# trifectatechfoundation/zlib-rs

Hardware: NVIDIA H100
Metric: deflate_level6_raw_input_throughput_silesia_small_tar (higher is better)
Workload: dtype u8

## Files before the change

zlib_rs_b200/csrc/zb_engine.cu:

```cuda
#include <cuda_runtime.h>
#include <stdio.h>
#include <stdlib.h>
#include <string.h>
#include <new>
#include "../../include/zb_engine.h"
#include "zb_kernels.cuh"
#include "zb_engine_internal.h"

namespace zb {

constexpr uint32_t kSlowSub9 = 24576;
constexpr uint32_t kTailTiles = 2;
constexpr uint32_t kTailSub = 512;

thread_local char g_err[256] = "";

static void set_err(const char *what, cudaError_t e)
{
    snprintf(g_err, sizeof g_err, "%s: %s", what, cudaGetErrorString(e));
}

#define CK(call)                                                  \
    do {                                                          \
        cudaError_t e_ = (call);                                  \
        if (e_ != cudaSuccess) { set_err(#call, e_); return ZB_E_CUDA; } \
    } while (0)

__global__ void k_match(JobBufs);
__global__ void k_skip(JobBufs);
__global__ void k_nxt(JobBufs);
__global__ void k_path_tiles(JobBufs);
__global__ void k_path_chain(JobBufs, uint32_t, uint32_t);
__global__ void k_path_groups(JobBufs, uint32_t, uint32_t, uint4 *, uint32_t *);
__global__ void k_path_chain2(JobBufs, uint32_t, uint32_t, const uint4 *, uint32_t *, uint32_t *);
__global__ void k_path_mark(JobBufs, const uint32_t *, const uint32_t *);
__global__ void k_iter_lists(JobBufs, uint32_t *, uint32_t *, uint32_t);
__global__ void k_emit(JobBufs);
__global__ void k_holes(JobBufs, uint32_t);
__global__ void k_holes_cmp(JobBufs, uint32_t, uint32_t);
__global__ void k_tail(JobBufs);
__global__ void k_block_hist(JobBufs, uint32_t *);
__global__ void k_build_blocks(JobBufs, const uint32_t *);
__global__ void k_scan_blocks(JobBufs);
__global__ void k_encode(JobBufs);
__global__ void k_finish(JobBufs, const uint32_t *);
__global__ void k_literal_syms(JobBufs);
__global__ void k_stored(JobBufs);
__global__ void k_links2_std(JobBufs, uint32_t);
__global__ void k_links2_roll(JobBufs, uint32_t);
__global__ void k_links_fix_std(JobBufs);
__global__ void k_links_fix_roll(JobBufs);
// ... 6 lines not shown
__global__ void k_links_dict_ghost_apply(JobBufs, const uint32_t *);
__global__ void k_bgzf_setup(BgzfJob, uint64_t);
__global__ void k_serial_low_members(JobBufs, BgzfJob);
__global__ void k_bgzf_medium(JobBufs, BgzfJob);
__global__ void k_bgzf_slow_steps(JobBufs, BgzfJob);
__global__ void k_bgzf_slow_walk(JobBufs, BgzfJob);
__global__ void k_bgzf_hist(JobBufs, BgzfJob, uint32_t *);
__global__ void k_bgzf_build(JobBufs, BgzfJob, const uint32_t *);
__global__ void k_bgzf_size(JobBufs, BgzfJob);
__global__ void k_bgzf_scan(JobBufs, BgzfJob);
__global__ void k_bgzf_encode(JobBufs, BgzfJob);
__global__ void k_bgzf_frame(JobBufs, BgzfJob);
__global__ void k_batch_stage(const uint8_t *, const uint64_t *, const uint8_t *, BgzfJob, uint8_t *, uint64_t);
__global__ void k_batch_dict_ghost(JobBufs, BgzfJob);

constexpr uint32_t kMatchSmemBytes = (kWSize + kMatchSub + 512) + (kWSize + kMatchSub) * 2 + ((kWSize + kMatchSub) / 32 + 1) * 4 * 4 + 8192;
constexpr uint32_t kPathSmemBytes = kPathTile * 4 * 3;
constexpr uint32_t kLinks2SmemBytes = 65536 * 2 + kLinkTile * 2 + kLinkTile + 64 + 2048;
constexpr uint32_t kSkipSmemBytes = 2 * kWSize * 2 + 2 * (2 * kWSize / 32) * 4 + 8192 + 64;
constexpr uint32_t kSlowSubMax = 24576;
constexpr uint32_t kSlowSmemBytes = (kWSize + kSlowSubMax + kSlowAhead) * 3;
constexpr uint32_t kChainSmemBytes = kChainChunkTiles * kPathHead * 8;
constexpr uint32_t kChain2MaxSmem = 200 * 1024;
constexpr uint32_t kSerialSmemBytes = (65536 + kWSize) * 2 + 35824 + 16;
constexpr uint32_t kSerialSmemQuick = 65536 * 2 + 65536 + 16;

int Engine::init(int dev)
{
    int n = 0;
    cudaError_t e = cudaGetDeviceCount(&n);
    if (e != cudaSuccess || n == 0) {
// ... 34 lines not shown
Engine::~Engine()
{
    if (device < 0) return;
    cudaSetDevice(device);
    for (auto &b : bufs) if (b.p) cudaFree(b.p);
    if (h_stage) cudaFreeHost(h_stage);
    if (h_info) cudaFreeHost(h_info);
    if (d_info) cudaFree(d_info);
    if (d_check) cudaFree(d_check);
    if (ev0) cudaEventDestroy(ev0);
    if (ev1) cudaEventDestroy(ev1);
    if (evf) cudaEventDestroy(evf);
    if (evt) cudaEventDestroy(evt);
    for (int i = 0; i < kUpChunks; i++) if (evc[i]) cudaEventDestroy(evc[i]);
    if (evk) cudaEventDestroy(evk);
    if (st2) cudaStreamDestroy(st2);
    if (st) cudaStreamDestroy(st);
}

void Engine::pbegin()
{
    if (!profile) return;
    if (!pev0) { cudaEventCreate(&pev0); cudaEventCreate(&pev1); }
    cudaEventRecord(pev0, st);
}

void Engine::pend(int phase, uint32_t nlaunch)
{
    if (!profile) return;
    cudaEventRecord(pev1, st);
// ... 119 lines not shown
    RES(S_SYMB, 40000 * 4, sym_base, uint32_t *)
    RES(S_BMAP, (size_t)nmt * 8192, bucket_map, uint32_t *)
    RES(S_LR, npad * 2, Lr, uint16_t *)
    RES(S_KEYS, npad * 2, keys, uint16_t *)
    RES(S_LLAST, (size_t)nmt * 65536 * 2, link_last, uint16_t *)
    RES(S_CSTATE, (size_t)(npt + 1) * 16, chain_state, uint4 *)
    uint32_t chainG = 16;
    while ((uint64_t)chainG * chainG < npt) chainG += 8;
    const uint32_t chain_groups = (npt + chainG - 1) / chainG;
    const uint32_t chain2_smem = chainG * kPathHead * 8 + chain_groups * kPathHead * 16 + chainG * 8;
    const bool chain2 = chain2_smem <= kChain2MaxSmem;
    if ((rc = reserve(S_GFN, (size_t)chain_groups * kPathHead * 16 + ((size_t)npt + 4) * 4, &p)) != ZB_OK) return rc;
    uint4 *d_gfn = static_cast<uint4 *>(p);
    uint32_t *d_mark_cnt = reinterpret_cast<uint32_t *>(d_gfn + (size_t)chain_groups * kPathHead);
    uint32_t *d_mark_list = d_mark_cnt + 4;
    auto launch_chain = [&](uint32_t first_tile) {
        if (chain2) {
            k_path_groups<<<chain_groups, 1024, chainG * kPathHead * 8, st>>>(jb, npt, chainG, d_gfn, d_mark_cnt);
            k_path_chain2<<<chain_groups, 1024, chain2_smem, st>>>(jb, npt, chainG, d_gfn, d_mark_list, d_mark_cnt);
            launches++;
        } else k_path_chain<<<1, 1024, kChainSmemBytes, st>>>(jb, npt, first_tile);
    };
    auto launch_mark = [&](uint32_t grid) {
        if (chain2) k_path_mark<<<grid < npt ? grid : npt, 1024, kPathSmemBytes, st>>>(jb, d_mark_list, d_mark_cnt);
        else k_path_mark<<<npt, 1024, kPathSmemBytes, st>>>(jb, nullptr, nullptr);
    };
    uint32_t *d_lists;
    const uint32_t max_list = N / 512 + 2;
    if ((rc = reserve(S_LISTS, ((size_t)max_list + npt + nmt + 8) * 4, &p)) != ZB_OK) return rc;
    d_lists = static_cast<uint32_t *>(p);
    RES(S_HDIFF, (size_t)nwords * 8, hdiff, uint32_t *)
    jb.hdiff_words = nwords;
    RES(S_HCOARSE, (size_t)(N >> 10) + 16, hcoarse, uint8_t *)
    RES(S_MCHG, (((size_t)N >> 8) + 16) * 4 + 64, mchg, uint8_t *)
    RES(S_BLOCKS, (size_t)max_blocks * sizeof(BlockDesc), blocks, BlockDesc *)
    RES(S_BBASE, (size_t)max_blocks * 4, block_base, uint32_t *)
    uint32_t *d_freq;
    if ((rc = reserve(S_FREQ, (size_t)max_blocks * 320 * 4, &p)) != ZB_OK) return rc;
    d_freq = static_cast<uint32_t *>(p);
    uint8_t *d_out;
    if (dst_dev && dst_cap >= out_cap) d_out = static_cast<uint8_t *>(dst);
    else { if ((rc = reserve(S_OUT, out_cap + 16, &p)) != ZB_OK) return rc; d_out = static_cast<uint8_t *>(p); }
    jb.out = d_out;
    jb.out_cap = out_cap;
    void *d_ck;
// ... 152 lines not shown
            if (!jb.slow_mode) CK(cudaMemcpyAsync(jb.Lr, jb.L, npad * 2, cudaMemcpyDeviceToDevice, st));
            pend(0, 1);
            if (jb.slow_mode) {
                if (n_in > 0) {
                    iters = 1;
                    pbegin();
                    if (jb.slow_mode == 2) k_rle<<<(N + 255) / 256, 256, 0, st>>>(jb);
                    else {
                        jb.match_sub = level >= 9 ? kSlowSub9 : level == 8 ? 4096u : 8192u;
                        k_slow<<<(N + jb.match_sub - 1) / jb.match_sub, 1024, (kWSize + jb.match_sub + kSlowAhead) * 3, st>>>(jb);
                    }
                    pend(1, 1);
                    if (profile) phase_ms[11] = phase_ms[1];
                    pbegin();
                    k_path_tiles<<<npt, 1024, kPathSmemBytes, st>>>(jb);
                    launch_chain(0);
                    launch_mark(npt);
                    pend(3, 3);
                    pbegin();
                    k_emit_slow<<<(N + 255) / 256, 256, 0, st>>>(jb);
                    pend(4, 1);
                    launches += 5;
                }
                pbegin();
                k_tail_slow<<<1, 32, 0, st>>>(jb);
                launches++;
                pend(5, 1);
            } else {
            if (jb.tail_start > 0) {
                uint32_t n_dirty = nmt;
                for (;;) {
                    iters++;
                    uint32_t mthreads = 1024;
                    if (iters == 1) jb.match_sub = 4096;
                    else if (n_dirty <= kTailTiles) { jb.match_sub = kTailSub; mthreads = 256; }
                    else {
                        const uint64_t per_cta = (uint64_t)n_dirty * kMatchTile / (4 * (uint64_t)device_sm_count());
                        jb.match_sub = per_cta >= 8192 ? 8192 : per_cta >= 4096 ? 4096 : per_cta >= 2048 ? 2048 : 1024;
                    }
                    uint32_t nsub = (N + jb.match_sub - 1) / jb.match_sub;
                    uint32_t n_ptiles = npt, first_ptile = 0;
                    jb.skip_list = nullptr;
                    jb.nxt_list = nullptr;
                    if (iters > 1) {
                        jb.skip_list = d_lists;
                        jb.nxt_list = d_lists + nmt + 8;
                        n_ptiles = h_info->n_ptiles ? h_info->n_ptiles : 1;
                        first_ptile = h_info->first_ptile;
                        nsub = (n_dirty ? n_dirty : 1) * (kMatchTile / jb.match_sub);
                        if (n_dirty) {
                            pbegin();
                            k_skip<<<n_dirty, 1024, kSkipSmemBytes, st>>>(jb);
                            pend(1, 1);
                            launches++;
                        }
                    }
                    const uint32_t msmem = (kWSize + jb.match_sub + 512) + (kWSize + jb.match_sub) * 2 +
                                           (iters > 1 ? ((kWSize + jb.match_sub) / 32 + 1) * 4 * 4 + 8192 : 64);
                    jb.use_bucket_map = iters > 1;
                    pbegin();
                    k_match<<<nsub, mthreads, msmem, st>>>(jb);
                    pend(1, 1);
                    if (profile && iters == 1) phase_ms[11] = phase_ms[1];
                    pbegin();
                    k_nxt<<<n_ptiles * (kPathTile / 1024), 1024, 0, st>>>(jb);
                    pend(2, 1);
                    pbegin();
                    k_path_tiles<<<n_ptiles, 1024, kPathSmemBytes, st>>>(jb);
                    launch_chain(first_ptile);
                    launch_mark(iters == 1 ? npt : 2 * n_ptiles + 16);
                    pend(3, 3);
                    pbegin();
                    k_holes<<<(nlists * kLongPerSub + 255) / 256, 256, 0, st>>>(jb, nlists);
                    k_holes_cmp<<<(nwords + 255) / 256, 256, 0, st>>>(jb, nwords, nmt);
                    pend(4, 2);
                    launches += 7;
                    k_iter_lists<<<1, 1024, 0, st>>>(jb, d_lists, d_lists + nmt + 8, npt);
                    launches++;
                    CK(cudaMemcpyAsync(h_info, d_info, sizeof(JobInfo), cudaMemcpyDeviceToHost, st));
                    CK(cudaStreamSynchronize(st));
                    if (h_info->error) { snprintf(g_err, sizeof g_err, "engine error flags 0x%x (parse)", h_info->error); return ZB_E_INTERNAL; }
                    if (getenv("ZB_DEBUG")) {
                        static unsigned long long last[3];
                        if (iters == 1) memset(last, 0, sizeof last);
                        const double ctas = (double)(h_info->dbg[0] - last[0]) + 1e-9;
                        fprintf(stderr, "iter %u dirty %u: ctas %llu stage %.1f walk %.1f kcyc/cta, holes_changed %u, sub %u first_tile %u chain %u\n",
                                iters, n_dirty, h_info->dbg[0] - last[0], (h_info->dbg[1] - last[1]) / 1e3 / ctas,
                                (h_info->dbg[2] - last[2]) / 1e3 / ctas, h_info->holes_changed, jb.match_sub, first_ptile, chain2 ? 2u : 1u);
                        memcpy(last, h_info->dbg, sizeof last);
                    }
                    if (!h_info->holes_changed) break;
                    n_dirty = h_info->n_dirty;
                    if (iters > N / 257u + 4096u) { snprintf(g_err, sizeof g_err, "hole iteration did not converge"); return ZB_E_INTERNAL; }
                }
            }
            CK(cudaEventRecord(evf, st));
            CK(cudaStreamWaitEvent(st2, evf, 0));
            k_tail<<<1, 32, 0, st2>>>(jb);
            launches++;
            CK(cudaEventRecord(evt, st2));
            if (jb.tail_start > 0) {
                pbegin();
                k_emit<<<(jb.tail_start + 255) / 256, 256, 0, st>>>(jb);
                launches++;
                pend(4, 1);
            }
            pbegin();
            CK(cudaStreamWaitEvent(st, evt, 0));
            pend(5, 1);
            }
        }
        CK(cudaMemcpyAsync(h_info, d_info, sizeof(JobInfo), cudaMemcpyDeviceToHost, st));
        CK(cudaStreamSynchronize(st));
        if (h_info->error) { snprintf(g_err, sizeof g_err, "engine error flags 0x%x (tail)", h_info->error); return ZB_E_INTERNAL; }
        const uint32_t nblocks = h_info->n_blocks;
        if (nblocks == 0 || nblocks > max_blocks) { snprintf(g_err, sizeof g_err, "bad block count %u", nblocks); return ZB_E_INTERNAL; }
        pbegin();
        k_block_hist<<<nblocks, 256, 0, st>>>(jb, d_freq);
        k_build_blocks<<<nblocks, 32, 0, st>>>(jb, d_freq);
        k_scan_blocks<<<1, 256, 0, st>>>(jb);
        pend(6, 3);
        pbegin();
        k_encode<<<nblocks, 1024, 0, st>>>(jb);
        k_finish<<<1, 32, 0, st>>>(jb, d_check);
        pend(7, 2);
        launches += 5;
    }
    CK(cudaMemcpyAsync(h_info, d_info, sizeof(JobInfo), cudaMemcpyDeviceToHost, st));
    CK(cudaStreamSynchronize(st));
    CK(cudaGetLastError());
    if (h_info->error) {
        if (h_info->error & 8u) return ZB_E_BUF;
        snprintf(g_err, sizeof g_err, "engine error flags 0x%x (encode)", h_info->error);
        return ZB_E_INTERNAL;
    }
    const uint64_t out_bytes = h_info->out_bytes;
    if (out_bytes > dst_cap) {
        res->out_bytes = out_bytes;
        return ZB_E_BUF;
    }
    if (d_out != dst) {
        pbegin();
        CK(cudaMemcpyAsync(dst, d_out, out_bytes, dst_dev ? cudaMemcpyDeviceToDevice : cudaMemcpyDeviceToHost, st));
        pend(10, 0);
    }
    CK(cudaEventRecord(ev1, st));
    CK(cudaStreamSynchronize(st));
    float ms = 0;
// ... 655 lines not shown
```

zlib_rs_b200/csrc/zb_engine_internal.h:

```cpp
#pragma once
#include <cuda_runtime.h>
#include <stddef.h>
#include <stdint.h>
#include <vector>
#include "../../include/zb_engine.h"
#include "zb_index.h"
#include "zb_kernels.cuh"

namespace zb {

extern thread_local char g_err[256];
size_t deflate_bound(size_t n);

enum { S_IN, S_L, S_HOLES, S_HOLESN, S_M, S_NXT, S_PEXIT, S_PCNT, S_SYMIDX, S_TENTRY, S_TSYMB, S_TDIRTY, S_SYMS, S_SYMB,
       S_BLOCKS, S_SCRATCH, S_FREQ, S_OUT, S_CK, S_INF0, S_INF1, S_PHEAD, S_SK, S_MARKN, S_LLIST, S_LCNT, S_BMAP, S_HDIFF, S_HCOARSE, S_CSTATE, S_LISTS, S_LR, S_LLAST, S_BBASE, S_MCHG, S_GFN, S_KEYS, S_SHARD,
       S_MEMT, S_MEMC,
       S_BGZF,
       S_BATCH,
       S_INDEX,
       S_INDEXW,
       S_COUNT };

struct ShardState {
    int phase = 0;
// ... 39 lines not shown
    Buf bufs[kSlots];
    void *h_stage = nullptr;
    size_t h_stage_cap = 0;
    JobInfo *h_info = nullptr, *d_info = nullptr;
    uint32_t *d_check = nullptr;
    void *d_inf_state = nullptr, *h_inf_state = nullptr;
    uint32_t launches = 0;
    uint8_t h_prime = 0;
    static constexpr int kPhases = 12;
    bool profile = false;
    float phase_ms[kPhases] = {0};
    uint32_t phase_launches[kPhases] = {0};
    cudaEvent_t pev0 = nullptr, pev1 = nullptr;
    void pbegin();
    void pend(int phase, uint32_t nlaunch);

    int init(int dev);
    int inflate_init();
    ~Engine();
    int reserve(int slot, size_t bytes, void **out);
    int stage(size_t bytes);
    int deflate(const void *src, size_t n, bool src_dev, void *dst, size_t dst_cap, bool dst_dev, int level, int strategy,
                int window_bits, uint32_t flags, zb_deflate_result *res, const void *dict = nullptr, size_t dict_len = 0);
    int deflate_bgzf(const void *src, size_t n, bool src_dev, void *dst, size_t dst_cap, bool dst_dev, int level, zb_deflate_result *res);
    int deflate_batch(const void *dict, size_t dict_len, const void *src, const uint64_t *src_off, size_t n_items, bool src_dev, void *dst,
                      size_t dst_cap, bool dst_dev, int level, int strategy, int window_bits, uint32_t flags, uint64_t *dst_off,
                      uint32_t *checks, zb_deflate_result *res);
    int members_reserve(JobBufs &jb, BgzfJob &bj, uint32_t nm, uint32_t S, size_t span, int level, size_t out_cap, uint32_t wrap,
                        uint32_t **d_freq);
    int members_launch(JobBufs &jb, BgzfJob &bj, int level, uint32_t *d_freq);
// ... 34 lines not shown
```

zlib_rs_b200/csrc/zb_kernels.cu:

```cuda
#include "zb_kernels.cuh"

namespace zb {

__constant__ HuffTables c_tab;

cudaError_t upload_tables()
{
    HuffTables t;
    init_tables(t);
    return cudaMemcpyToSymbol(c_tab, &t, sizeof t);
}

struct GAcc {
    const uint8_t *data;
    uint32_t N;
    const uint16_t *L;
    const uint32_t *holes;
    const uint32_t *M;
    uint32_t w = kWSize;
    __device__ __forceinline__ uint32_t byte(uint32_t y) const
    {
        while (y >= N) {
            if (y < 2 * w) return 0;
            y -= w;
// ... 154 lines not shown
}

__global__ void __launch_bounds__(1024) k_links2_std(JobBufs jb, uint32_t tile0) { links2_body<false>(jb, tile0); }
__global__ void __launch_bounds__(1024) k_links2_roll(JobBufs jb, uint32_t tile0) { links2_body<true>(jb, tile0); }
__global__ void __launch_bounds__(256) k_links_fix_std(JobBufs jb) { links_fix_body<false>(jb); }
__global__ void __launch_bounds__(256) k_links_fix_roll(JobBufs jb) { links_fix_body<true>(jb); }

constexpr uint32_t kSkipSpan = 2 * kWSize;
__global__ void __launch_bounds__(1024) k_skip(JobBufs jb)
{
    extern __shared__ __align__(16) uint8_t smem[];
    uint16_t *sL = reinterpret_cast<uint16_t *>(smem);
    uint32_t *sh = reinterpret_cast<uint32_t *>(smem + kSkipSpan * 2);
    uint32_t *sf = sh + kSkipSpan / 32;
    uint32_t *sbm = sf + kSkipSpan / 32;
    const uint32_t tile = jb.skip_list ? jb.skip_list[blockIdx.x] : blockIdx.x;
    const uint32_t ts = tile * kMatchTile;
    if (ts >= jb.N) return;
    const uint32_t te = min(ts + kMatchTile, jb.N);
    const uint32_t ws = ts >= kWSize ? ts - kWSize : 0;
    const uint32_t span = te - ws, tid = threadIdx.x;
    const uint32_t md = jb.wsize - kMinLookahead;
    {
        const uint4 *ls = reinterpret_cast<const uint4 *>(jb.L + ws);
        uint4 *ld = reinterpret_cast<uint4 *>(sL);
        for (uint32_t i = tid; i < (span + 7) / 8; i += 1024) ld[i] = ls[i];
        for (uint32_t i = tid; i < (span + 31) / 32; i += 1024) sh[i] = jb.holes[(ws >> 5) + i];
        const uint32_t *bm1 = jb.bucket_map + (size_t)tile * 2048, *bm0 = tile ? bm1 - 2048 : bm1;
        for (uint32_t i = tid; i < 2048; i += 1024) sbm[i] = bm0[i] | bm1[i];
    }
// ... 280 lines not shown
                        }
                    }
                }
            }
        }
    }
}

__global__ void __launch_bounds__(1024, 2) k_match(JobBufs jb)
{
    extern __shared__ __align__(16) uint8_t smem[];
    __shared__ uint32_t s_next;
    __shared__ __align__(8) unsigned long long s_mbar;
    const uint32_t sub = jb.match_sub;
    const uint32_t per_tile = kMatchTile / sub;
    const uint32_t ts = (jb.skip_list ? jb.skip_list[blockIdx.x / per_tile] * per_tile + blockIdx.x % per_tile : blockIdx.x) * sub;
    if (ts >= jb.N) return;
    {
        const uint32_t t0 = ts / kMatchTile, t1 = (min(ts + sub, jb.N) - 1) / kMatchTile;
        if (!jb.tile_dirty[t0] && !jb.tile_dirty[t1]) return;
    }
    const uint32_t data_bytes = kWSize + sub + 512;
    uint8_t *sdata = smem;
    uint16_t *sL = reinterpret_cast<uint16_t *>(smem + data_bytes);
    uint32_t *sh = reinterpret_cast<uint32_t *>(smem + data_bytes + (kWSize + sub) * 2);
    uint32_t *sbm = sh;
    const uint32_t wmax = (kWSize + sub) / 32 + 1;
    uint32_t *sdel = sbm + 2048, *pdel = sdel + wmax, *sadd = pdel + wmax, *padd = sadd + wmax;
    __shared__ uint32_t s_wsum[32];
    const uint32_t N = jb.N;
// ... 116 lines not shown
    }
}

constexpr uint32_t kMacroReach = 22016;

__device__ __forceinline__ bool path_tile_dirty(const JobBufs &jb, uint32_t pt)
{
    const uint32_t m0 = (pt * kPathTile) / kMatchTile;
    uint32_t m1 = ((pt + 1) * kPathTile + kMacroReach - 1) / kMatchTile;
    if (m1 >= jb.nmt) m1 = jb.nmt - 1;
    bool d = false;
    for (uint32_t m = m0; m <= m1; m++) d = d || jb.tile_dirty[m];
    return d;
}

__global__ void __launch_bounds__(1024) k_nxt(JobBufs jb)
{
    constexpr uint32_t per = kPathTile / 1024;
    const uint32_t tile = jb.nxt_list ? jb.nxt_list[blockIdx.x / per] : blockIdx.x / per;
    if (!path_tile_dirty(jb, tile)) return;
    const uint32_t p = tile * kPathTile + (blockIdx.x % per) * 1024 + threadIdx.x;
    if (p >= jb.tail_start) return;
    if (jb.use_bucket_map) {
        const uint32_t old = jb.nxt[p];
        const uint32_t b0 = p >> 6, b1 = min(p + (old & 0xffffu), jb.N) >> 6;
        bool chg = false;
        for (uint32_t b = b0; b <= b1; b++) chg = chg || jb.mchg[b];
        if (!chg) return;
    }
    GAcc a{jb.in, jb.N, jb.L, jb.holes, jb.M, jb.wsize};
    const uint32_t long_len = 16 * jb.lp.lazy;
    uint32_t ns = 0, nlong = 0, lpos = 0, llen = 0;
    auto see = [&](const Sym &s) {
// ... 49 lines not shown
            v.x = p < jb.tail_start ? jb.nxt[p] : t;
            v.y = p + 1 < jb.tail_start ? jb.nxt[p + 1] : t;
            v.z = p + 2 < jb.tail_start ? jb.nxt[p + 2] : t;
            v.w = t;
        }
        dst[g] = v;
    }
}

__global__ void __launch_bounds__(1024) k_path_tiles(JobBufs jb)
{
    extern __shared__ __align__(16) uint8_t smem[];
    uint32_t *nx = reinterpret_cast<uint32_t *>(smem);
    uint32_t *ex = nx + kPathTile;
    uint32_t *cn = ex + kPathTile;
    const uint32_t tile = jb.nxt_list ? jb.nxt_list[blockIdx.x] : blockIdx.x;
    const uint32_t tbeg = tile * kPathTile;
    if (!path_tile_dirty(jb, tile)) return;
    path_load(jb, tbeg, nx);
    __syncthreads();
    const uint32_t warp = threadIdx.x >> 5, lane = threadIdx.x & 31;
    constexpr uint32_t kExitSub = 1024, nsub = kPathTile / kExitSub;
    for (uint32_t s = warp; s < nsub; s += blockDim.x / 32) path_subtile(nx, ex, cn, s * kExitSub, (s + 1) * kExitSub, lane);
    __syncthreads();
    for (int32_t j = (int32_t)nsub - 2; j >= 0; j--) {
        for (uint32_t i = threadIdx.x; i < kExitSub; i += blockDim.x) {
            const uint32_t p = (uint32_t)j * kExitSub + i;
            uint32_t t = ex[p];
            if (!(t & kStuck) && t < kPathTile) { cn[p] += cn[t]; ex[p] = ex[t]; }
        }
// ... 6 lines not shown
        if (p < jb.tail_start) {
            jb.pexit[p] = xa;
            jb.pcnt[p] = cn[i];
        }
        if (i < kPathHead) jb.phead[(size_t)tile * kPathHead + i] = make_uint2(xa, cn[i]);
    }
}

constexpr uint32_t kChainChunk = kChainChunkTiles;
__global__ void __launch_bounds__(1024) k_path_chain(JobBufs jb, uint32_t ntiles, uint32_t first_tile)
{
    extern __shared__ __align__(16) uint8_t smem[];
    uint2 *hd = reinterpret_cast<uint2 *>(smem);
    __shared__ uint32_t s_e, s_base, s_done, s_tail;
    __shared__ uint32_t c_entry[kChainChunk], c_base[kChainChunk];
    if (threadIdx.x == 0) {
        if (first_tile == 0) { s_e = jb.start; s_base = 0; s_done = jb.tail_start == 0; s_tail = jb.start; }
        else { const uint4 v = jb.chain_state[first_tile]; s_e = v.x; s_base = v.y; s_done = v.z; s_tail = v.w; }
    }
    for (uint32_t t = threadIdx.x; t < first_tile; t += blockDim.x) jb.mark_needed[t] = 0;
    __syncthreads();
    for (uint32_t c0 = first_tile; c0 < ntiles; c0 += kChainChunk) {
        const uint32_t nt = min(kChainChunk, ntiles - c0);
        for (uint32_t i = threadIdx.x; i < nt * kPathHead; i += blockDim.x) hd[i] = jb.phead[(size_t)c0 * kPathHead + i];
        __syncthreads();
        if (threadIdx.x == 0) {
            uint32_t e = s_e, base = s_base;
            bool done = s_done != 0;
            uint32_t tail_entry = s_tail;
            for (uint32_t k = 0; k < nt; k++) {
// ... 271 lines not shown
                diff &= diff - 1;
                if (y + 4 <= jb.N) {
                    const uint8_t *q = jb.in + y;
                    const uint32_t h = hash_u32((uint32_t)q[0] | ((uint32_t)q[1] << 8) | ((uint32_t)q[2] << 16) | ((uint32_t)q[3] << 24));
                    atomicOr(&sb[h >> 5], 1u << (h & 31));
                }
            }
        }
        jb.holes_new[w] = 0;
    }
    __syncthreads();
    uint32_t *bm = jb.bucket_map + (size_t)((blockIdx.x * blockDim.x * 32) / kMatchTile) * 2048;
    for (uint32_t i = threadIdx.x; i < 2048; i += blockDim.x) if (sb[i]) atomicOr(&bm[i], sb[i]);
}

__global__ void __launch_bounds__(1024) k_iter_lists(JobBufs jb, uint32_t *skip_list, uint32_t *path_list, uint32_t npt)
{
    __shared__ uint32_t s_wsum[32], s_total, s_first;
    const uint32_t tid = threadIdx.x, lane = tid & 31, warp = tid >> 5;
    if (tid == 0) s_first = 0xffffffffu;
    uint32_t base = 0;
    for (int which = 0; which < 2; which++) {
        const uint32_t n = which ? npt : jb.nmt;
        uint32_t *out = which ? path_list : skip_list;
        base = 0;
        for (uint32_t c0 = 0; c0 < n; c0 += 1024) {
            const uint32_t i = c0 + tid;
            const bool d = i < n && (which ? path_tile_dirty(jb, i) : jb.tile_dirty[i] != 0);
            const uint32_t m = __ballot_sync(0xffffffffu, d);
            __syncthreads();
            if (lane == 0) s_wsum[warp] = __popc(m);
// ... 8 lines not shown
            }
            __syncthreads();
            if (d) {
                out[base + s_wsum[warp] + __popc(m & ((1u << lane) - 1u))] = i;
                if (which) atomicMin(&s_first, i);
            }
            base += s_total;
        }
        __syncthreads();
        if (tid == 0) {
            if (which) { jb.info->n_ptiles = base; jb.info->first_ptile = s_first == 0xffffffffu ? 0u : s_first; }
            else jb.info->n_dirty = base;
        }
        if (tid == 0 && base == 0) out[0] = 0;
    }
}

struct GAccW {
    GAcc g;
    uint32_t w;
    __device__ __forceinline__ uint32_t byte(uint32_t y) const
    {
        while (y >= g.N) {
            if (y < 2 * w) return 0;
            y -= w;
        }
        return g.data[y];
    }
    __device__ __forceinline__ uint32_t link(uint32_t y) const { return g.link(y); }
    __device__ __forceinline__ bool inserted(uint32_t y) const { return g.inserted(y); }
// ... 36 lines not shown
        if (s.dist == 0) atomicAdd(&lf[s.lc], 1u);
        else {
            atomicAdd(&lf[257 + c_tab.length_code[s.lc]], 1u);
            atomicAdd(&df[d_code(c_tab, s.dist - 1u)], 1u);
        }
    }
    __syncthreads();
    for (uint32_t i = threadIdx.x; i < kLCodes; i += blockDim.x) fb[i] = lf[i];
    if (threadIdx.x < kDCodes) fb[kLCodes + threadIdx.x] = df[threadIdx.x];
}

__global__ void __launch_bounds__(256) k_block_hist(JobBufs jb, uint32_t *freq )
{
    const uint32_t b = blockIdx.x;
    const uint32_t nsyms = jb.info->n_syms, nblocks = jb.info->n_blocks;
    const uint32_t begin = b * jb.block_syms;
    const uint32_t count = (b + 1 < nblocks) ? jb.block_syms : nsyms - begin;
    block_hist_body(jb.syms, begin, count, freq + b * 320);
    if (threadIdx.x == 0) {
        BlockDesc &bd = jb.blocks[b];
        const bool last = b + 1 == nblocks;
        bd.sym_begin = begin;
        bd.sym_count = count;
        bd.last = last && !jb.not_last;
        const uint32_t start = begin == 0 ? jb.start : sym_end(jb.syms[begin - 1]);
        const uint32_t end = last ? jb.N : sym_end(jb.syms[begin + count - 1]);
        bd.in_start = start;
        bd.in_len = end - start;
        uint32_t Bf;
        if (last) Bf = jb.info->final_base;
// ... 306 lines not shown
    const uint64_t w = pos >> 5;
    const uint32_t sh = (uint32_t)(pos & 31);
    atomicOr(&out32[w], (uint32_t)(val << sh));
    if (sh + n > 32) {
        atomicOr(&out32[w + 1], (uint32_t)(val >> (32 - sh)));
        if (sh + n > 64) atomicOr(&out32[w + 2], (uint32_t)(val >> (64 - sh)));
    }
}

constexpr uint32_t kScanChunk = 1024;
__global__ void __launch_bounds__(256) k_scan_blocks(JobBufs jb)
{
    __shared__ uint64_t s_bits[kScanChunk];
    __shared__ uint64_t s_base[kScanChunk];
    __shared__ uint64_t s_bit;
    const uint32_t nb = jb.info->n_blocks;
    if (threadIdx.x == 0) s_bit = 8ull * jb.hdr_len + jb.prime_bits;
    for (uint32_t c0 = 0; c0 < nb; c0 += kScanChunk) {
        const uint32_t nc = min(kScanChunk, nb - c0);
        for (uint32_t i = threadIdx.x; i < nc; i += blockDim.x) {
            const BlockDesc &bd = jb.blocks[c0 + i];
            s_bits[i] = bd.type == 0 ? (1ull << 63) | (uint16_t)bd.in_len : (uint64_t)bd.hdr_bits + bd.body_bits;
        }
        __syncthreads();
        if (threadIdx.x == 0) {
            uint64_t bit = s_bit;
            for (uint32_t i = 0; i < nc; i++) {
                s_base[i] = bit;
                const uint64_t v = s_bits[i];
                bit = (v >> 63) ? ((bit + 3 + 7) & ~7ull) + 32 + 8ull * (v & 0xffffu) : bit + v;
// ... 110 lines not shown
        __syncthreads();
        uint64_t pos = bd.bit_base + bd.hdr_bits + round_bits + (incl - mybits) + (warp ? warp_sum[warp - 1] : 0);
#pragma unroll
        for (uint32_t j = 0; j < kSymsPerThread; j++) {
            or_bits(out32, pos, vals[j], lens[j]);
            pos += lens[j];
        }
        round_bits += warp_sum[31];
        __syncthreads();
    }
    if (tid == blockDim.x - 1 && round_bits != bd.body_bits) atomicOr(error, 16u);
}

__global__ void __launch_bounds__(1024) k_encode(JobBufs jb)
{
    if (jb.info->error) return;
    encode_body(jb.blocks[blockIdx.x], jb.syms, jb.in, jb.out, &jb.info->error);
}

__global__ void __launch_bounds__(256) k_bgzf_hist(JobBufs jb, BgzfJob bj, uint32_t *freq)
{
    const uint32_t b = blockIdx.x, m = b / kBgzfMaxBlocks, k = b % kBgzfMaxBlocks;
    const JobInfo &mi = bj.minfo[m];
    const uint32_t nsyms = mi.n_syms, nblocks = mi.n_blocks;
    if (k >= nblocks) return;
    const uint32_t base = (uint32_t)bj.moff[m], len = bj.pstart + bj.mlen[m];
    const Sym *syms = jb.syms + base;
    const uint32_t begin = k * jb.block_syms;
    const uint32_t count = k + 1 < nblocks ? jb.block_syms : nsyms - begin;
    block_hist_body(syms, begin, count, freq + (size_t)b * 320);
    if (threadIdx.x == 0) {
// ... 104 lines not shown
```

zlib_rs_b200/csrc/zb_kernels.cuh:

```cuda
#pragma once
#include <cuda_runtime.h>
#include "zb_core.h"
#include "zb_huff.h"
#include "zb_slow.h"
#include "zb_bgzf.h"

namespace zb {

constexpr uint32_t kLinkTile = 32768;
constexpr uint32_t kMatchTile = 32768;
constexpr uint32_t kMatchSub = 8192;
constexpr uint32_t kPathTile = 16384;
constexpr uint32_t kPathSub = 256;
constexpr uint32_t kLongPerSub = 4;
constexpr uint32_t kPathHead = 64;
constexpr uint32_t kChainChunkTiles = 320;
constexpr uint32_t kNxtTail = 0x80000000u;
constexpr uint32_t kNxtLong = 0x40000000u;
constexpr uint32_t kNxtLong258 = 0x20000000u;
constexpr uint32_t kSymsPerThread = 16;
constexpr uint32_t kSlowAhead = 1024;

__device__ __forceinline__ uint32_t sld_u8(uint32_t a) { uint32_t v; asm volatile("ld.shared.u8 %0, [%1];" : "=r"(v) : "r"(a)); return v; }
__device__ __forceinline__ uint32_t sld_u16(uint32_t a) { uint32_t v; asm volatile("ld.shared.u16 %0, [%1];" : "=r"(v) : "r"(a)); return v; }
// ... 7 lines not shown
struct JobInfo {
    uint32_t n_mid_syms;
    uint32_t tail_entry;
    uint32_t n_syms;
    uint32_t final_base;
    uint32_t holes_changed;
    uint32_t n_dirty, n_ptiles, first_ptile;
    uint32_t n_blocks;
    uint32_t data_type;
    uint32_t error;
    uint64_t total_bits;
    uint64_t out_bytes;
    uint32_t adler;
    uint64_t marker_byte;
    unsigned long long dbg[3];
};

struct JobBufs {
    const uint8_t *in;
    uint32_t N;
    uint32_t start;
    uint32_t tail_start;
    uint16_t *L;
    uint16_t *SK;
    uint32_t *hdiff;
    uint32_t hdiff_words;
    uint8_t *hcoarse;
    uint8_t *mchg;
    uint32_t *holes;
    uint32_t *holes_new;
    uint32_t *M;
// ... 59 lines not shown
    uint64_t *moff;
    uint32_t *mlen;
    uint32_t *mcheck;
    uint32_t *mbytes;
    uint64_t *mout;
    uint32_t *mstored;
    JobInfo *minfo;
    BgzfCtl *ctl;
    uint32_t pstart;
    uint32_t fdict;
    const uint32_t *dictid;
};

cudaError_t upload_tables();
int device_sm_count();
cudaError_t launch_adler32(const uint8_t *d_buf, uint64_t len, uint32_t start, void *d_scratch, size_t scratch_bytes, uint32_t *d_out,
                           cudaStream_t st);
cudaError_t launch_crc32(const uint8_t *d_buf, uint64_t len, uint32_t start, void *d_scratch, size_t scratch_bytes, uint32_t *d_out,
                         cudaStream_t st);
cudaError_t launch_crc32_segments(const uint8_t *d_buf, const uint64_t *d_off, const uint32_t *d_len, uint32_t nseg, uint32_t *d_crc,
                                  cudaStream_t st);
cudaError_t launch_crc32_join(const uint32_t *d_crc, const uint32_t *d_len, const uint32_t *d_count, uint32_t *d_out, cudaStream_t st);
cudaError_t launch_adler32_segments(const uint8_t *d_buf, const uint64_t *d_off, const uint32_t *d_len, uint32_t nseg, uint32_t *d_adler,
                                    cudaStream_t st);

}
```

Measured before the change: 1.598.

## Run hole iteration loop on device via CUDA graph conditional nodes

Replaces the host-driven hole-refinement loop, which synchronised and copied JobInfo back after every iteration, with a cached CUDA graph. The graph uses a while-conditional node and per-match-class if-branches, and k_iter_lists sets the conditions on the device. It also removes the host sync before block encoding by launching the encode kernels with max_blocks and letting them early-exit based on device-side n_blocks. The trade-off is over-provisioned grids, since kernels are launched with upper-bound sizes and exit early, plus graph build cost whenever the key changes.

```diff
diff --git a/zlib_rs_b200/csrc/zb_engine.cu b/zlib_rs_b200/csrc/zb_engine.cu
--- a/zlib_rs_b200/csrc/zb_engine.cu
+++ b/zlib_rs_b200/csrc/zb_engine.cu
@@ -10,8 +10,6 @@
 namespace zb {
 
 constexpr uint32_t kSlowSub9 = 24576;
-constexpr uint32_t kTailTiles = 2;
-constexpr uint32_t kTailSub = 512;
 
 thread_local char g_err[256] = "";
 
@@ -34,7 +32,7 @@
 __global__ void k_path_groups(JobBufs, uint32_t, uint32_t, uint4 *, uint32_t *);
 __global__ void k_path_chain2(JobBufs, uint32_t, uint32_t, const uint4 *, uint32_t *, uint32_t *);
 __global__ void k_path_mark(JobBufs, const uint32_t *, const uint32_t *);
-__global__ void k_iter_lists(JobBufs, uint32_t *, uint32_t *, uint32_t);
+__global__ void k_iter_lists(JobBufs, uint32_t *, uint32_t *, uint32_t, IterCtl);
 __global__ void k_emit(JobBufs);
 __global__ void k_holes(JobBufs, uint32_t);
 __global__ void k_holes_cmp(JobBufs, uint32_t, uint32_t);
@@ -71,7 +69,11 @@
 __global__ void k_batch_stage(const uint8_t *, const uint64_t *, const uint8_t *, BgzfJob, uint8_t *, uint64_t);
 __global__ void k_batch_dict_ghost(JobBufs, BgzfJob);
 
-constexpr uint32_t kMatchSmemBytes = (kWSize + kMatchSub + 512) + (kWSize + kMatchSub) * 2 + ((kWSize + kMatchSub) / 32 + 1) * 4 * 4 + 8192;
+constexpr uint32_t match_smem(uint32_t sub, bool later)
+{
+    return (kWSize + sub + 512) + (kWSize + sub) * 2 + (later ? ((kWSize + sub) / 32 + 1) * 4 * 4 + 8192 : 64);
+}
+constexpr uint32_t kMatchSmemBytes = match_smem(kMatchSub, true);
 constexpr uint32_t kPathSmemBytes = kPathTile * 4 * 3;
 constexpr uint32_t kLinks2SmemBytes = 65536 * 2 + kLinkTile * 2 + kLinkTile + 64 + 2048;
 constexpr uint32_t kSkipSmemBytes = 2 * kWSize * 2 + 2 * (2 * kWSize / 32) * 4 + 8192 + 64;
@@ -136,6 +138,9 @@
     if (evt) cudaEventDestroy(evt);
     for (int i = 0; i < kUpChunks; i++) if (evc[i]) cudaEventDestroy(evc[i]);
     if (evk) cudaEventDestroy(evk);
+    if (hg_exec) cudaGraphExecDestroy(hg_exec);
+    if (hg) cudaGraphDestroy(hg);
+    if (hg_st) cudaStreamDestroy(hg_st);
     if (st2) cudaStreamDestroy(st2);
     if (st) cudaStreamDestroy(st);
 }
@@ -285,21 +290,95 @@
     uint4 *d_gfn = static_cast<uint4 *>(p);
     uint32_t *d_mark_cnt = reinterpret_cast<uint32_t *>(d_gfn + (size_t)chain_groups * kPathHead);
     uint32_t *d_mark_list = d_mark_cnt + 4;
-    auto launch_chain = [&](uint32_t first_tile) {
+    auto launch_chain = [&](const JobBufs &j, cudaStream_t s, uint32_t first_tile) {
         if (chain2) {
-            k_path_groups<<<chain_groups, 1024, chainG * kPathHead * 8, st>>>(jb, npt, chainG, d_gfn, d_mark_cnt);
-            k_path_chain2<<<chain_groups, 1024, chain2_smem, st>>>(jb, npt, chainG, d_gfn, d_mark_list, d_mark_cnt);
-            launches++;
-        } else k_path_chain<<<1, 1024, kChainSmemBytes, st>>>(jb, npt, first_tile);
+            k_path_groups<<<chain_groups, 1024, chainG * kPathHead * 8, s>>>(j, npt, chainG, d_gfn, d_mark_cnt);
+            k_path_chain2<<<chain_groups, 1024, chain2_smem, s>>>(j, npt, chainG, d_gfn, d_mark_list, d_mark_cnt);
+        } else k_path_chain<<<1, 1024, kChainSmemBytes, s>>>(j, npt, first_tile);
     };
-    auto launch_mark = [&](uint32_t grid) {
-        if (chain2) k_path_mark<<<grid < npt ? grid : npt, 1024, kPathSmemBytes, st>>>(jb, d_mark_list, d_mark_cnt);
-        else k_path_mark<<<npt, 1024, kPathSmemBytes, st>>>(jb, nullptr, nullptr);
+    auto launch_mark = [&](const JobBufs &j, cudaStream_t s, uint32_t grid) {
+        if (chain2) k_path_mark<<<grid < npt ? grid : npt, 1024, kPathSmemBytes, s>>>(j, d_mark_list, d_mark_cnt);
+        else k_path_mark<<<npt, 1024, kPathSmemBytes, s>>>(j, nullptr, nullptr);
     };
     uint32_t *d_lists;
     const uint32_t max_list = N / 512 + 2;
     if ((rc = reserve(S_LISTS, ((size_t)max_list + npt + nmt + 8) * 4, &p)) != ZB_OK) return rc;
     d_lists = static_cast<uint32_t *>(p);
+    const uint32_t max_iters = N / 257u + 4096u;
+    bool graph_iters = false;
+    auto hole_graph = [&](uint32_t sms) -> int {
+        JobBufs jg = jb;
+        jg.out = nullptr;
+        jg.out_cap = 0;
+        jg.skip_list = d_lists;
+        jg.nxt_list = d_lists + nmt + 8;
+        jg.use_bucket_map = 1;
+        jg.match_sub = 0;
+        HoleGraphKey key;
+        memset(&key, 0, sizeof key);
+        key.jb = jg;
+        key.npt = npt; key.nlists = nlists; key.nwords = nwords; key.sms = sms; key.chain2 = chain2;
+        key.lists = d_lists; key.gfn = d_gfn;
+        if (hg_valid && memcmp(&key, &hg_key, sizeof key) == 0) return ZB_OK;
+        hg_valid = false;
+        if (hg_exec) { cudaGraphExecDestroy(hg_exec); hg_exec = nullptr; }
+        if (hg) { cudaGraphDestroy(hg); hg = nullptr; }
+        if (!hg_st) CK(cudaStreamCreateWithFlags(&hg_st, cudaStreamNonBlocking));
+        IterCtl ctl{};
+        ctl.graph = 1;
+        ctl.sms = sms;
+        ctl.max_iters = max_iters;
+        uint32_t dmax[kMatchClasses] = {1, 1, 1, 1, 1};
+        for (uint32_t d = 1; d <= nmt; d++) { const int c = match_class(d, sms); if (d > dmax[c]) dmax[c] = d; }
+        const uint32_t reach = path_tiles_per_match_tile(nmt, npt);
+        for (int c = 0; c < kMatchClasses; c++) ctl.ptile_bound[c] = (uint64_t)dmax[c] * reach < npt ? dmax[c] * reach : npt;
+        CK(cudaGraphCreate(&hg, 0));
+        cudaGraphConditionalHandle h;
+        CK(cudaGraphConditionalHandleCreate(&h, hg, 1, cudaGraphCondAssignDefault));
+        ctl.loop = h;
+        cudaGraphNodeParams wp = {cudaGraphNodeTypeConditional};
+        wp.conditional.handle = h;
+        wp.conditional.type = cudaGraphCondTypeWhile;
+        wp.conditional.size = 1;
+        cudaGraphNode_t node;
+        CK(cudaGraphAddNode(&node, hg, nullptr, 0, &wp));
+        cudaGraph_t body = wp.conditional.phGraph_out[0];
+        for (int c = 0; c < kMatchClasses; c++) {
+            CK(cudaGraphConditionalHandleCreate(&h, body, 0, cudaGraphCondAssignDefault));
+            ctl.cls[c] = h;
+        }
+        CK(cudaStreamBeginCaptureToGraph(hg_st, body, nullptr, nullptr, 0, cudaStreamCaptureModeThreadLocal));
+        k_iter_lists<<<1, 1024, 0, hg_st>>>(jg, d_lists, d_lists + nmt + 8, npt, ctl);
+        CK(cudaStreamEndCapture(hg_st, &body));
+        cudaGraphNode_t lists_node;
+        size_t nn = 1;
+        CK(cudaGraphGetNodes(body, &lists_node, &nn));
+        for (int c = 0; c < kMatchClasses; c++) {
+            cudaGraphNodeParams ip = {cudaGraphNodeTypeConditional};
+            ip.conditional.handle = ctl.cls[c];
+            ip.conditional.type = cudaGraphCondTypeIf;
+            ip.conditional.size = 1;
+            CK(cudaGraphAddNode(&node, body, &lists_node, 1, &ip));
+            cudaGraph_t br = ip.conditional.phGraph_out[0];
+            JobBufs jc = jg;
+            jc.match_sub = match_class_sub(c);
+            const uint32_t D = dmax[c], P = ctl.ptile_bound[c];
+            CK(cudaStreamBeginCaptureToGraph(hg_st, br, nullptr, nullptr, 0, cudaStreamCaptureModeThreadLocal));
+            k_skip<<<D, 1024, kSkipSmemBytes, hg_st>>>(jc);
+            k_match<<<D * (kMatchTile / jc.match_sub), c == 0 ? 256 : 1024, match_smem(jc.match_sub, true), hg_st>>>(jc);
+            k_nxt<<<P * (kPathTile / 1024), 1024, 0, hg_st>>>(jc);
+            k_path_tiles<<<P, 1024, kPathSmemBytes, hg_st>>>(jc);
+            launch_chain(jc, hg_st, kFirstFromInfo);
+            launch_mark(jc, hg_st, 2 * P + 16);
+            k_holes<<<(nlists * kLongPerSub + 255) / 256, 256, 0, hg_st>>>(jc, nlists);
+            k_holes_cmp<<<(nwords + 255) / 256, 256, 0, hg_st>>>(jc, nwords, nmt);
+            CK(cudaStreamEndCapture(hg_st, &br));
+        }
+        CK(cudaGraphInstantiate(&hg_exec, hg, 0));
+        hg_key = key;
+        hg_valid = true;
+        return ZB_OK;
+    };
     RES(S_HDIFF, (size_t)nwords * 8, hdiff, uint32_t *)
     jb.hdiff_words = nwords;
     RES(S_HCOARSE, (size_t)(N >> 10) + 16, hcoarse, uint8_t *)
@@ -482,8 +561,9 @@
                     if (profile) phase_ms[11] = phase_ms[1];
                     pbegin();
                     k_path_tiles<<<npt, 1024, kPathSmemBytes, st>>>(jb);
-                    launch_chain(0);
-                    launch_mark(npt);
+                    launch_chain(jb, st, 0);
+                    launch_mark(jb, st, npt);
+                    if (chain2) launches++;
                     pend(3, 3);
                     pbegin();
                     k_emit_slow<<<(N + 255) / 256, 256, 0, st>>>(jb);
@@ -496,15 +576,17 @@
                 pend(5, 1);
             } else {
             if (jb.tail_start > 0) {
+                const bool host_loop = profile || getenv("ZB_DEBUG") != nullptr;
+                const uint32_t sms = (uint32_t)device_sm_count();
                 uint32_t n_dirty = nmt;
                 for (;;) {
                     iters++;
                     uint32_t mthreads = 1024;
                     if (iters == 1) jb.match_sub = 4096;
-                    else if (n_dirty <= kTailTiles) { jb.match_sub = kTailSub; mthreads = 256; }
                     else {
-                        const uint64_t per_cta = (uint64_t)n_dirty * kMatchTile / (4 * (uint64_t)device_sm_count());
-                        jb.match_sub = per_cta >= 8192 ? 8192 : per_cta >= 4096 ? 4096 : per_cta >= 2048 ? 2048 : 1024;
+                        const int c = match_class(n_dirty, sms);
+                        jb.match_sub = match_class_sub(c);
+                        if (c == 0) mthreads = 256;
                     }
                     uint32_t nsub = (N + jb.match_sub - 1) / jb.match_sub;
                     uint32_t n_ptiles = npt, first_ptile = 0;
@@ -523,11 +605,9 @@
                             launches++;
                         }
                     }
-                    const uint32_t msmem = (kWSize + jb.match_sub + 512) + (kWSize + jb.match_sub) * 2 +
-                                           (iters > 1 ? ((kWSize + jb.match_sub) / 32 + 1) * 4 * 4 + 8192 : 64);
                     jb.use_bucket_map = iters > 1;
                     pbegin();
-                    k_match<<<nsub, mthreads, msmem, st>>>(jb);
+                    k_match<<<nsub, mthreads, match_smem(jb.match_sub, iters > 1), st>>>(jb);
                     pend(1, 1);
                     if (profile && iters == 1) phase_ms[11] = phase_ms[1];
                     pbegin();
@@ -535,15 +615,16 @@
                     pend(2, 1);
                     pbegin();
                     k_path_tiles<<<n_ptiles, 1024, kPathSmemBytes, st>>>(jb);
-                    launch_chain(first_ptile);
-                    launch_mark(iters == 1 ? npt : 2 * n_ptiles + 16);
+                    launch_chain(jb, st, first_ptile);
+                    launch_mark(jb, st, iters == 1 ? npt : 2 * n_ptiles + 16);
                     pend(3, 3);
                     pbegin();
                     k_holes<<<(nlists * kLongPerSub + 255) / 256, 256, 0, st>>>(jb, nlists);
                     k_holes_cmp<<<(nwords + 255) / 256, 256, 0, st>>>(jb, nwords, nmt);
                     pend(4, 2);
-                    launches += 7;
-                    k_iter_lists<<<1, 1024, 0, st>>>(jb, d_lists, d_lists + nmt + 8, npt);
+                    launches += chain2 ? 8 : 7;
+                    if (!host_loop) break;
+                    k_iter_lists<<<1, 1024, 0, st>>>(jb, d_lists, d_lists + nmt + 8, npt, IterCtl{});
                     launches++;
                     CK(cudaMemcpyAsync(h_info, d_info, sizeof(JobInfo), cudaMemcpyDeviceToHost, st));
                     CK(cudaStreamSynchronize(st));
@@ -559,7 +640,12 @@
                     }
                     if (!h_info->holes_changed) break;
                     n_dirty = h_info->n_dirty;
-                    if (iters > N / 257u + 4096u) { snprintf(g_err, sizeof g_err, "hole iteration did not converge"); return ZB_E_INTERNAL; }
+                    if (iters > max_iters) { snprintf(g_err, sizeof g_err, "hole iteration did not converge"); return ZB_E_INTERNAL; }
+                }
+                if (!host_loop) {
+                    if ((rc = hole_graph(sms)) != ZB_OK) return rc;
+                    CK(cudaGraphLaunch(hg_exec, st));
+                    graph_iters = true;
                 }
             }
             CK(cudaEventRecord(evf, st));
@@ -578,18 +664,13 @@
             pend(5, 1);
             }
         }
-        CK(cudaMemcpyAsync(h_info, d_info, sizeof(JobInfo), cudaMemcpyDeviceToHost, st));
-        CK(cudaStreamSynchronize(st));
-        if (h_info->error) { snprintf(g_err, sizeof g_err, "engine error flags 0x%x (tail)", h_info->error); return ZB_E_INTERNAL; }
-        const uint32_t nblocks = h_info->n_blocks;
-        if (nblocks == 0 || nblocks > max_blocks) { snprintf(g_err, sizeof g_err, "bad block count %u", nblocks); return ZB_E_INTERNAL; }
         pbegin();
-        k_block_hist<<<nblocks, 256, 0, st>>>(jb, d_freq);
-        k_build_blocks<<<nblocks, 32, 0, st>>>(jb, d_freq);
+        k_block_hist<<<max_blocks, 256, 0, st>>>(jb, d_freq);
+        k_build_blocks<<<max_blocks, 32, 0, st>>>(jb, d_freq);
         k_scan_blocks<<<1, 256, 0, st>>>(jb);
         pend(6, 3);
         pbegin();
-        k_encode<<<nblocks, 1024, 0, st>>>(jb);
+        k_encode<<<max_blocks, 1024, 0, st>>>(jb);
         k_finish<<<1, 32, 0, st>>>(jb, d_check);
         pend(7, 2);
         launches += 5;
@@ -597,9 +678,15 @@
     CK(cudaMemcpyAsync(h_info, d_info, sizeof(JobInfo), cudaMemcpyDeviceToHost, st));
     CK(cudaStreamSynchronize(st));
     CK(cudaGetLastError());
+    if (graph_iters) {
+        iters = h_info->iters;
+        launches += 1 + (iters - 1) * (chain2 ? 10u : 9u);
+    }
     if (h_info->error) {
         if (h_info->error & 8u) return ZB_E_BUF;
-        snprintf(g_err, sizeof g_err, "engine error flags 0x%x (encode)", h_info->error);
+        if (h_info->error & kErrNoConverge) snprintf(g_err, sizeof g_err, "hole iteration did not converge");
+        else if (h_info->error & kErrBlockCount) snprintf(g_err, sizeof g_err, "bad block count %u", h_info->n_blocks);
+        else snprintf(g_err, sizeof g_err, "engine error flags 0x%x", h_info->error);
         return ZB_E_INTERNAL;
     }
     const uint64_t out_bytes = h_info->out_bytes;
diff --git a/zlib_rs_b200/csrc/zb_engine_internal.h b/zlib_rs_b200/csrc/zb_engine_internal.h
--- a/zlib_rs_b200/csrc/zb_engine_internal.h
+++ b/zlib_rs_b200/csrc/zb_engine_internal.h
@@ -77,6 +77,16 @@
     cudaEvent_t pev0 = nullptr, pev1 = nullptr;
     void pbegin();
     void pend(int phase, uint32_t nlaunch);
+    struct HoleGraphKey {
+        JobBufs jb;
+        uint32_t npt, nlists, nwords, sms, chain2;
+        const void *lists, *gfn;
+    };
+    HoleGraphKey hg_key;
+    bool hg_valid = false;
+    cudaGraph_t hg = nullptr;
+    cudaGraphExec_t hg_exec = nullptr;
+    cudaStream_t hg_st = nullptr;
 
     int init(int dev);
     int inflate_init();
diff --git a/zlib_rs_b200/csrc/zb_kernels.cu b/zlib_rs_b200/csrc/zb_kernels.cu
--- a/zlib_rs_b200/csrc/zb_kernels.cu
+++ b/zlib_rs_b200/csrc/zb_kernels.cu
@@ -1,3 +1,4 @@
+#include <vector>
 #include "zb_kernels.cuh"
 
 namespace zb {
@@ -192,6 +193,7 @@
     uint32_t *sh = reinterpret_cast<uint32_t *>(smem + kSkipSpan * 2);
     uint32_t *sf = sh + kSkipSpan / 32;
     uint32_t *sbm = sf + kSkipSpan / 32;
+    if (jb.skip_list && blockIdx.x >= jb.info->n_dirty) return;
     const uint32_t tile = jb.skip_list ? jb.skip_list[blockIdx.x] : blockIdx.x;
     const uint32_t ts = tile * kMatchTile;
     if (ts >= jb.N) return;
@@ -502,6 +504,7 @@
     __shared__ __align__(8) unsigned long long s_mbar;
     const uint32_t sub = jb.match_sub;
     const uint32_t per_tile = kMatchTile / sub;
+    if (jb.skip_list && blockIdx.x / per_tile >= max(jb.info->n_dirty, 1u)) return;
     const uint32_t ts = (jb.skip_list ? jb.skip_list[blockIdx.x / per_tile] * per_tile + blockIdx.x % per_tile : blockIdx.x) * sub;
     if (ts >= jb.N) return;
     {
@@ -648,9 +651,23 @@
     return d;
 }
 
+uint32_t path_tiles_per_match_tile(uint32_t nmt, uint32_t npt)
+{
+    std::vector<uint32_t> cover(nmt, 0);
+    for (uint32_t pt = 0; pt < npt; pt++) {
+        const uint32_t m0 = (uint32_t)((uint64_t)pt * kPathTile / kMatchTile);
+        const uint32_t m1 = (uint32_t)(((uint64_t)(pt + 1) * kPathTile + kMacroReach - 1) / kMatchTile);
+        for (uint32_t m = m0; m <= m1 && m < nmt; m++) cover[m]++;
+    }
+    uint32_t most = 1;
+    for (uint32_t v : cover) most = v > most ? v : most;
+    return most;
+}
+
 __global__ void __launch_bounds__(1024) k_nxt(JobBufs jb)
 {
     constexpr uint32_t per = kPathTile / 1024;
+    if (jb.nxt_list && blockIdx.x / per >= max(jb.info->n_ptiles, 1u)) return;
     const uint32_t tile = jb.nxt_list ? jb.nxt_list[blockIdx.x / per] : blockIdx.x / per;
     if (!path_tile_dirty(jb, tile)) return;
     const uint32_t p = tile * kPathTile + (blockIdx.x % per) * 1024 + threadIdx.x;
@@ -730,6 +747,7 @@
     uint32_t *nx = reinterpret_cast<uint32_t *>(smem);
     uint32_t *ex = nx + kPathTile;
     uint32_t *cn = ex + kPathTile;
+    if (jb.nxt_list && blockIdx.x >= max(jb.info->n_ptiles, 1u)) return;
     const uint32_t tile = jb.nxt_list ? jb.nxt_list[blockIdx.x] : blockIdx.x;
     const uint32_t tbeg = tile * kPathTile;
     if (!path_tile_dirty(jb, tile)) return;
@@ -766,6 +784,7 @@
     uint2 *hd = reinterpret_cast<uint2 *>(smem);
     __shared__ uint32_t s_e, s_base, s_done, s_tail;
     __shared__ uint32_t c_entry[kChainChunk], c_base[kChainChunk];
+    if (first_tile == kFirstFromInfo) first_tile = jb.info->first_ptile;
     if (threadIdx.x == 0) {
         if (first_tile == 0) { s_e = jb.start; s_base = 0; s_done = jb.tail_start == 0; s_tail = jb.start; }
         else { const uint4 v = jb.chain_state[first_tile]; s_e = v.x; s_base = v.y; s_done = v.z; s_tail = v.w; }
@@ -1067,7 +1086,7 @@
     for (uint32_t i = threadIdx.x; i < 2048; i += blockDim.x) if (sb[i]) atomicOr(&bm[i], sb[i]);
 }
 
-__global__ void __launch_bounds__(1024) k_iter_lists(JobBufs jb, uint32_t *skip_list, uint32_t *path_list, uint32_t npt)
+__global__ void __launch_bounds__(1024) k_iter_lists(JobBufs jb, uint32_t *skip_list, uint32_t *path_list, uint32_t npt, IterCtl ctl)
 {
     __shared__ uint32_t s_wsum[32], s_total, s_first;
     const uint32_t tid = threadIdx.x, lane = tid & 31, warp = tid >> 5;
@@ -1106,6 +1125,15 @@
         }
         if (tid == 0 && base == 0) out[0] = 0;
     }
+    if (tid != 0) return;
+    const uint32_t iters = ++jb.info->iters;
+    if (!ctl.graph) return;
+    bool go = jb.info->holes_changed != 0;
+    if (go && iters > ctl.max_iters) { atomicOr(&jb.info->error, kErrNoConverge); go = false; }
+    const int c = match_class(jb.info->n_dirty, ctl.sms);
+    if (go && max(jb.info->n_ptiles, 1u) > ctl.ptile_bound[c]) { atomicOr(&jb.info->error, kErrListBound); go = false; }
+    cudaGraphSetConditional(ctl.loop, go ? 1u : 0u);
+    for (int k = 0; k < kMatchClasses; k++) cudaGraphSetConditional(ctl.cls[k], go && k == c ? 1u : 0u);
 }
 
 struct GAccW {
@@ -1172,6 +1200,9 @@
 {
     const uint32_t b = blockIdx.x;
     const uint32_t nsyms = jb.info->n_syms, nblocks = jb.info->n_blocks;
+    const bool bad = nblocks == 0 || nblocks > gridDim.x;
+    if (bad && b == 0 && threadIdx.x == 0) atomicOr(&jb.info->error, kErrBlockCount);
+    if (bad || b >= nblocks || jb.info->error) return;
     const uint32_t begin = b * jb.block_syms;
     const uint32_t count = (b + 1 < nblocks) ? jb.block_syms : nsyms - begin;
     block_hist_body(jb.syms, begin, count, freq + b * 320);
@@ -1508,6 +1539,7 @@
     __shared__ uint64_t s_bits[kScanChunk];
     __shared__ uint64_t s_base[kScanChunk];
     __shared__ uint64_t s_bit;
+    if (jb.info->error) return;
     const uint32_t nb = jb.info->n_blocks;
     if (threadIdx.x == 0) s_bit = 8ull * jb.hdr_len + jb.prime_bits;
     for (uint32_t c0 = 0; c0 < nb; c0 += kScanChunk) {
@@ -1648,7 +1680,7 @@
 
 __global__ void __launch_bounds__(1024) k_encode(JobBufs jb)
 {
-    if (jb.info->error) return;
+    if (jb.info->error || blockIdx.x >= jb.info->n_blocks) return;
     encode_body(jb.blocks[blockIdx.x], jb.syms, jb.in, jb.out, &jb.info->error);
 }
 
diff --git a/zlib_rs_b200/csrc/zb_kernels.cuh b/zlib_rs_b200/csrc/zb_kernels.cuh
--- a/zlib_rs_b200/csrc/zb_kernels.cuh
+++ b/zlib_rs_b200/csrc/zb_kernels.cuh
@@ -45,7 +45,32 @@
     uint32_t adler;
     uint64_t marker_byte;
     unsigned long long dbg[3];
+    uint32_t iters;
 };
+constexpr uint32_t kErrBlockCount = 64u;
+constexpr uint32_t kErrNoConverge = 256u;
+constexpr uint32_t kErrListBound = 512u;
+
+constexpr uint32_t kTailTiles = 2;
+constexpr uint32_t kTailSub = 512;
+constexpr int kMatchClasses = 5;
+__host__ __device__ inline int match_class(uint32_t n_dirty, uint32_t sms)
+{
+    if (n_dirty <= kTailTiles) return 0;
+    const uint64_t per_cta = (uint64_t)n_dirty * kMatchTile / (4 * (uint64_t)sms);
+    return per_cta >= 8192 ? 4 : per_cta >= 4096 ? 3 : per_cta >= 2048 ? 2 : 1;
+}
+__host__ __device__ inline uint32_t match_class_sub(int c) { return 512u << c; }
+
+struct IterCtl {
+    uint32_t graph;
+    uint32_t sms;
+    uint32_t max_iters;
+    uint32_t ptile_bound[kMatchClasses];
+    unsigned long long loop;
+    unsigned long long cls[kMatchClasses];
+};
+constexpr uint32_t kFirstFromInfo = 0xffffffffu;
 
 struct JobBufs {
     const uint8_t *in;
@@ -135,6 +160,7 @@
 
 cudaError_t upload_tables();
 int device_sm_count();
+uint32_t path_tiles_per_match_tile(uint32_t nmt, uint32_t npt);
 cudaError_t launch_adler32(const uint8_t *d_buf, uint64_t len, uint32_t start, void *d_scratch, size_t scratch_bytes, uint32_t *d_out,
                            cudaStream_t st);
 cudaError_t launch_crc32(const uint8_t *d_buf, uint64_t len, uint32_t start, void *d_scratch, size_t scratch_bytes, uint32_t *d_out,
```

New measurement: 1.601 (median of 6 runs). No clear change (+0.2%).
